# blasif/cocons

Measured on AMD Instinct MI355X. Metric: -2loglik evals/sec (dense cov_rns + Cholesky/solve/log-det, fp64) at n=10000, higher is better.
Workload: dtype f64

## Files before the change

cocons_amd/csrc/api.hip:

```cpp
#include <hip/hip_runtime.h>
#include <limits.h>
#include <math.h>
#include <stdarg.h>
#include <stdint.h>
#include <stdio.h>
#include <stdlib.h>
#include <string.h>
#include <unistd.h>
#include <time.h>
#include <dlfcn.h>
#include <rccl/rccl.h>

#include <algorithm>
#include <limits>
#include <memory>
#include <mutex>
#include <string>
#include <thread>
#include <vector>

#include "kernels.h"
#include "../../include/cocons_hip_diag.h"
#include "matern_device.hpp"

using namespace cocons;

static thread_local std::string g_err;

static int fail(int code, const char *fmt, ...)
{
    char buf[512];
    va_list ap;
    va_start(ap, fmt);
    vsnprintf(buf, sizeof buf, fmt, ap);
    va_end(ap);
    g_err = buf;
    return code;
}

#define HIPCHK(expr)                                                              \
    do {                                                                          \
        hipError_t e__ = (expr);                                                  \
        if (e__ != hipSuccess) {                                                  \
            char b__[512];                                                        \
            snprintf(b__, sizeof b__, "%s failed: %s (%s:%d)", #expr,             \
                     hipGetErrorString(e__), __FILE__, __LINE__);                 \
            g_err = b__;                                                          \
            return -100 - (int)e__;                                               \
        }                                                                         \
    } while (0)

extern "C" const char *cocons_last_error(void) { return g_err.c_str(); }
extern "C" int cocons_abi_version(void) { return 1; }

extern "C" int cocons_device_count(void)
{
    int n = 0;
    hipError_t e = hipGetDeviceCount(&n);
    if (e != hipSuccess) { g_err = hipGetErrorString(e); return -1; }
    return n;
}

extern "C" double cocons_sumsmoothlone(const double *x, int len, double lambda, double alpha)
{
    double sum = 0;
    for (int w = 0; w < len; ++w) {
        if (std::abs(x[w]) > 1e-4)
            sum = sum + std::abs(x[w]);
        else
            sum = sum + std::pow(alpha, -1) * (std::log(1 + std::exp(-alpha * x[w])) + std::log(1 + std::exp(alpha * x[w])));
    }
// ... 1464 lines not shown
    return 0;
}

static int enqueue_eval_impl(cocons_fit *f, const double *theta, const double *mean, bool use_trend,
                             const double *xb, int nxb, std::vector<hipEvent_t> *ev_upd, bool stage_events)
{
    const int nrhs = f->r + nxb;
    f->nrhs_cur = nrhs;
    const int was_clean = f->border_clean;
    const double *was_A = f->dA;
    if (int rc = fit_alloc_matrix(f, nrhs)) return rc;
    const bool zero_rest = !(was_clean == nrhs && was_A == f->dA);
    f->border_pending = nrhs;
    if (stage_events) hipEventRecord(f->ev[0], f->stream);
    if (int rc = reset_info(f)) return rc;
    if (f->taper_nnz > 0) { if (int rc = assemble_sigma_taper(f, theta)) return rc; }
    else assemble_sigma(f, theta, 0, 0, f->npad);
    const bool slots = f->nslot >= nrhs && f->nslot > 0;
    FactorView fv = main_view(f);
    if (slots) fv.mt = fv.nt;
    else fv.trim = (f->rhs_act - nrhs >= 64) ? 1 : 0;
    fv.dag_ok = true;
    if (engine_wanted(f, fv))
        if (int rc = engine_start(f, fv)) return rc;
    assemble_rhs(f, mean, use_trend, xb, nxb, 0, f->npad, zero_rest, slots);
    if (stage_events) hipEventRecord(f->ev[1], f->stream);
    if (int rc = factorize(f, fv, ev_upd)) return rc;
    if (stage_events) hipEventRecord(f->ev[2], f->stream);
    launch_finalize(f->dA, f->lda, f->n, slots ? f->n : f->npad, nrhs, f->dout, f->stream, f->skew, f->npad,
                    f->dag_used ? f->dP : nullptr, f->dag_used ? 2 * TILE * f->dag_nsteps : 0);
    HIPCHK(hipMemcpyAsync(f->hinfo, f->dinfo, (size_t)(2 + nrhs * nrhs) * sizeof(double),
                          hipMemcpyDeviceToHost, f->stream));
    if (stage_events) hipEventRecord(f->ev[3], f->stream);
    HIPCHK(hipGetLastError());
    return 0;
}

static void debug_abort_report(cocons_fit *f)
{
    fprintf(stderr, "cocons: hand-off time-out, code 0x%x\n", f->hinfo[1]);
    const unsigned cls = abort_class((unsigned)f->hinfo[1]);
    if (!f->dag_used || !f->ddag || cls < ABORT_DAG_FIRST || cls > ABORT_DAG_LAST) return;
    unsigned rec[7] = {0, 0, 0, 0, 0, 0, 0}, now = 0, qn = 0;
    hipMemcpyAsync(rec, f->ddag + 8, sizeof rec, hipMemcpyDeviceToHost, f->stream);
    hipStreamSynchronize(f->stream);
    if (rec[2] < f->ddag.count()) hipMemcpyAsync(&now, f->ddag + rec[2], sizeof now, hipMemcpyDeviceToHost, f->stream);
    hipMemcpyAsync(&qn, f->ddag, sizeof qn, hipMemcpyDeviceToHost, f->stream);
    hipStreamSynchronize(f->stream);
    fprintf(stderr, "cocons: DAG wait: task %u (of %u, counter now %u) code 0x%x waited for word %u >= %u, saw %u, holds %u now; "
            "%.1f ms, %u polls\n", rec[0], f->dag_ntasks, qn, rec[1], rec[2], rec[3], rec[4], now, rec[5] * 1e-5, rec[6]);
    if (const char *dump = getenv("COCONS_DEBUG_ABORT_DUMP")) {
        static int ndump = 0;
        char path[512];
        snprintf(path, sizeof path, "%s.%d", dump, ndump++);
        if (FILE *fp = fopen(path, "wb")) {
            const unsigned ntr = f->dag_trace_tasks ? 1u : 0u;
            unsigned hdr[16] = {0xDA6D0001u, (unsigned)f->nt, (unsigned)f->dag_nsteps, f->dag_ntasks, (unsigned)f->ddag.count(),
                                (unsigned)f->flags_cap, ntr, (unsigned)f->hinfo[1], qn, now, 0, 0, 0, 0, 0, 0};
            fwrite(hdr, sizeof hdr, 1, fp);
            fwrite(rec, sizeof rec, 1, fp);
            std::vector<DagStepHost> sh((size_t)f->dag_nsteps);
            hipMemcpyAsync(sh.data(), f->ddag_steps, sh.size() * sizeof(DagStepHost), hipMemcpyDeviceToHost, f->stream);
            std::vector<unsigned> w((size_t)f->ddag.count()), fl(4 * (size_t)f->flags_cap + 64);
            hipMemcpyAsync(w.data(), f->ddag, w.size() * sizeof(unsigned), hipMemcpyDeviceToHost, f->stream);
            hipMemcpyAsync(fl.data(), f->dflags, fl.size() * sizeof(unsigned), hipMemcpyDeviceToHost, f->stream);
            hipStreamSynchronize(f->stream);
// ... 1195 lines not shown
    pa.pad_diag = f->nslot > 0 ? 1e300 : 1.0;
    pa.own_world = world; pa.own_rank = rank; pa.own_group = shard_group();
    launch_pair_sym(ms.mode, false, pa, f->stream);
    const int mt = f->nt + f->rhs_act / TILE;
    if (shard_owner(f->nt / PT, world) == rank)
        assemble_rhs(f, mean, true, nullptr, 0, 0, f->npad);
    launch_front_identity(f->dA, f->lda, f->pad0, mt * TILE, f->stream);
    HIPCHK(hipGetLastError());
    return 0;
}

static int shard_factor_diag(cocons_fit *f, int k)
{
    ShardState *S = f->shard.get();
    const int t = k * PT, w = S->plan.ncols[k] / TILE;
    hipStream_t s = f->stream;
    double *A = f->dA, *q0 = f->dinv, *q1 = f->dinv + 2048;
    if (engine_enabled() && f->flags_cap >= t + w) {
        unsigned *in = f->dflags, *out = f->dflags + f->flags_cap, *xr = f->dflags + 2 * (size_t)f->flags_cap;
        HIPCHK(hipMemsetD32Async((hipDeviceptr_t)(in + t), 7, (size_t)w, s));
        const bool pair = w == 2 && tun().engine_pair && f->dmbox && f->smb_off >= ((size_t)f->nt + 2) * ENGINE_MBOX_DOUBLES;
        launch_potrf_engine(A, f->lda, t, t + w, f->dinv, f->dinfo, in, out, xr, (unsigned *)(f->dinfo + 1),
                            f->dflags + 3 * (size_t)f->flags_cap, s, nullptr, nullptr, 0, nullptr,
                            pair ? f->dmbox : nullptr);
    } else {
        launch_potrf_tile(A, f->lda, t * TILE, q0, f->dinfo, s);
        if (w == 2) {
            launch_trsm_tile(A, f->lda, t * TILE, (t + 1) * TILE, (t + 2) * TILE, q0, s);
            launch_update(A, f->lda, t * TILE, TILE, t + 1, t + 2, t + 1, t + 2, true, s);
            launch_potrf_tile(A, f->lda, (t + 1) * TILE, q1, f->dinfo, s);
        }
    }
    (void)q1;
    double *L = S->lkk[k & 1];
    HIPCHK(hipMemcpy2DAsync(L, (size_t)PT * TILE * sizeof(double), A + (size_t)t * TILE + (size_t)t * TILE * f->lda,
                            f->lda * sizeof(double), (size_t)w * TILE * sizeof(double), (size_t)w * TILE,
                            hipMemcpyDeviceToDevice, s));
    HIPCHK(hipMemcpyAsync(L + (size_t)PT * TILE * PT * TILE, f->dinv, 2 * 2048 * sizeof(double), hipMemcpyDeviceToDevice, s));
    HIPCHK(hipEventRecord(S->ev_main_L, s));
    return 0;
}

static bool shard_comm2()
{
    static const int v = [] { const char *e = getenv("COCONS_SHARD_COMM2"); return e ? atoi(e) : 0; }();
    return v != 0;
}

static int coll_prepare(cocons_fit *f)
{
    if (!f->cstream) HIPCHK(hipStreamCreateWithFlags(&f->cstream, hipStreamNonBlocking));
    if (!f->cstream_l) {
        const bool own = shard_comm2() && (f->coll_kind == 2 || (f->coll_kind == 1 && f->comm_l && f->comm_l != f->comm));
        if (own) HIPCHK(hipStreamCreateWithFlags(&f->cstream_l, hipStreamNonBlocking));
        else f->cstream_l = f->cstream;
    }
    if (!f->dcoll) HIPCHK(f->dcoll.alloc((size_t)(2 + (COCONS_P_MAX + f->r) * (COCONS_P_MAX + f->r))));
    return 0;
}

extern "C" int cocons_comm_unique_id(void *id_out)
{
    if (!id_out) return fail(-1, "cocons_comm_unique_id: null argument");
    RcclApi *R = rccl_api();
    if (!R) return -1;
    ncclUniqueId id;
// ... 92 lines not shown
    const int W = f->coll_world, rank = f->coll_rank, G = shard_group();
    const int t = k * PT, w = P.ncols[k] / TILE, tn = t + w;
    const int mt = P.mt;
    hipStream_t s = f->stream;
    double *A = f->dA;
    if (rank != shard_owner(k, W)) {
        HIPCHK(hipStreamWaitEvent(s, S->ev_comm_L[k & 1], 0));
        const double *L = S->lkk[k & 1];
        HIPCHK(hipMemcpy2DAsync(A + (size_t)t * TILE + (size_t)t * TILE * f->lda, f->lda * sizeof(double), L,
                                (size_t)PT * TILE * sizeof(double), (size_t)w * TILE * sizeof(double), (size_t)w * TILE,
                                hipMemcpyDeviceToDevice, s));
        HIPCHK(hipMemcpyAsync(f->dinv, L + (size_t)PT * TILE * PT * TILE, 2 * 2048 * sizeof(double), hipMemcpyDeviceToDevice, s));
        HIPCHK(hipEventRecord(S->ev_main_U[k & 1], s));
        S->unpacked[k & 1] = true;
    }
    if (tn >= mt) return 0;
    if (P.cnt[(size_t)k * W + rank] > 0) {
        launch_trsm_tile(A, f->lda, t * TILE, tn * TILE, mt * TILE, f->dinv, s, nullptr, nullptr, -1, 0, W, rank, G);
        if (w == 2) {
            launch_update_from(A, f->lda, A + (size_t)t * TILE * f->lda, f->lda, TILE, tn, mt, t + 1, t + 2, false, s, G, W, rank);
            launch_trsm_tile(A, f->lda, (t + 1) * TILE, tn * TILE, mt * TILE, f->dinv + 2048, s, nullptr, nullptr, -1, 0, W, rank, G);
        }
    }
    if (tn >= P.nt) return 0;
    if (k + 1 < nb && rank == shard_owner(k + 1, W)) {
        const int w1 = P.ncols[k + 1] / TILE;
        launch_update(A, f->lda, t * TILE, w * TILE, tn, tn + w1, tn, tn + w1, true, s);
        if (int rc = shard_factor_diag(f, k + 1)) return rc;
    }
    const long long slot = (long long)P.srows[k] * P.ncols[k];
    launch_pack_rows(A, f->lda, t * TILE, w * TILE, f->xbuf[k & 1], (size_t)P.srows[k], S->d_pmap + (size_t)k * 2 * mt, P.tlo[k],
                     2 * mt, slot * rank, slot * (rank + 1), s);
    HIPCHK(hipEventRecord(S->ev_main_X[k & 1], s));
    HIPCHK(hipGetLastError());
    return 0;
}

static int shard_step_post(cocons_fit *f, int k, int nb)
{
    ShardState *S = f->shard.get();
    const ShardPlan &P = S->plan;
    const int W = f->coll_world, rank = f->coll_rank, G = shard_group();
    const int t = k * PT, w = P.ncols[k] / TILE, tn = t + w;
    if (tn >= P.nt) return 0;
    HIPCHK(hipStreamWaitEvent(f->stream, S->ev_comm_X[k & 1], 0));
    if (P.cnt[(size_t)k * W + rank] > 0) {
        const bool ahead = k + 1 < nb && rank == shard_owner(k + 1, W);
        const int skip_lo = ahead ? 2 * tn : 0, skip_hi = ahead ? 2 * (tn + P.ncols[k + 1] / TILE) : 0;
        launch_update_from(f->dA, f->lda, f->xbuf[k & 1], (size_t)P.srows[k], w * TILE, tn, P.mt, tn, P.nt, true, f->stream,
                           G, W, rank, nullptr, -1, nullptr, nullptr, nullptr, -1, 0, 0, 0, 0,
                           S->d_pmap + (size_t)k * 2 * P.mt, skip_lo, skip_hi);
    }
    HIPCHK(hipGetLastError());
    return 0;
}

static int shard_finish(cocons_fit *f, double *partial, int *info)
{
    const int nr = f->nrhs_cur, len = 1 + nr * nr;
    for (int i = 0; i < len; ++i) partial[i] = 0.0;
    const bool mine = shard_owner(f->nt / PT, f->coll_world) == f->coll_rank;
    if (mine) {
        launch_finalize(f->dA, f->lda, f->n, f->npad, nr, f->dout, f->stream);
        HIPCHK(hipMemcpyAsync(f->hout, f->dout, (size_t)len * sizeof(double), hipMemcpyDeviceToHost, f->stream));
    }
    HIPCHK(hipMemcpyAsync(f->hinfo, f->dinfo, 2 * sizeof(int), hipMemcpyDeviceToHost, f->stream));
    HIPCHK(hipStreamSynchronize(f->stream));
    if (mine) for (int i = 0; i < len; ++i) partial[i] = f->hout[i];
    if (info) *info = *f->hinfo;
    return 0;
}

static int sharded_eval_impl(cocons_fit *f, const double *theta, const double *mean, double *sum_logliks, double *parts);

static int sharded_eval(cocons_fit *f, const double *theta, const double *mean, double *sum_logliks, double *parts)
{
    const int rc = sharded_eval_impl(f, theta, mean, sum_logliks, parts);
    if (rc < 0 && f->coll_kind == 1 && f->comm && f->coll_world > 1) {
        const std::string keep = g_err;
        RcclApi *R = rccl_api();
        if (R && f->comm_l && f->comm_l != f->comm) (void)R->CommAbort(f->comm_l);
        if (R) (void)R->CommAbort(f->comm);
        f->comm = nullptr; f->comm_l = nullptr;
        f->coll_kind = -1;
        g_err = keep + " (communicator aborted)";
// ... 343 lines not shown
                                 hipMemcpyDeviceToDevice, M) != hipSuccess) return fail(-100, tiles_failed);
        }
    }
    HIPCHK_AT("cocons_debug_dag_replay", dcmp.alloc(2));
    const size_t T64 = 2 * (size_t)fv.mt;
    unsigned *in = f->dflags, *outw = f->dflags + f->flags_cap, *xr = f->dflags + 2 * (size_t)f->flags_cap;
    unsigned *abort_word = (unsigned *)(f->dinfo + 1);
    unsigned *queue = f->ddag, *tdone = f->ddag + 64, *pdone = tdone + T64 * (T64 + 1) / 2;
    unsigned *pall = pdone + ((size_t)f->dag_nsteps + 2) * T64;
    unsigned *dcount = pall + (size_t)f->dag_nsteps + 64;
    f->upd_flops = 0.0;
    f->nrhs_cur = nrhs;
    for (int s2 = 0; s2 < f->dag_nsteps; ++s2) count_update_flops(f, 2, 2 * s2 + 2);
    const double flops = f->upd_flops;
    HIPCHK_AT("cocons_debug_dag_replay", hipEventCreate(&ev.a));
    HIPCHK_AT("cocons_debug_dag_replay", hipEventCreate(&ev.b));
    double ms_sum = 0.0;
    for (int it = 0; it < reps; ++it) {
        if (int rc = reset_info(f)) return rc;
        assemble_sigma(f, theta, 0, 0, f->npad);
        assemble_rhs(f, mean, true, nullptr, 0, 0, f->npad, true, slots);
        launch_front_identity(fv.A, fv.lda, f->pad0, fv.mt * TILE, M);
        panel_ops(f, fv, 0, M);
        HIPCHK_AT("cocons_debug_dag_replay", hipMemsetAsync(f->ddag, 0, f->ddag.count() * sizeof(unsigned), M));
        HIPCHK_AT("cocons_debug_dag_replay", hipMemsetD32Async((hipDeviceptr_t)f->dflags, 0x3fffffff, 3 * (size_t)f->flags_cap, M));
        unsigned *alive_w = f->dflags + 3 * (size_t)f->flags_cap;
        static const unsigned pair_on_xcd0 = 2u;
        HIPCHK_AT("cocons_debug_dag_replay", hipMemcpyAsync(alive_w + 16, &pair_on_xcd0, sizeof(unsigned), hipMemcpyHostToDevice, M));
        HIPCHK_AT("cocons_debug_dag_replay", hipEventRecord(ev.a, M));
        launch_dag(fv.A, fv.lda, f->dP, f->dWt, f->ddag_steps, f->dag_nsteps, f->dag_ntasks, queue, tdone,
                   pdone, (int)T64, pall, f->dpart, dcount, in, outw, xr, abort_word, M, nullptr, alive_w, dag_xcc_quota(), nullptr,
                   f->dag_have_ftab ? f->ddag_ftab : nullptr, f->dag_xcd_g, f->ddag + f->ddag_xcnt_off);
        HIPCHK_AT("cocons_debug_dag_replay", hipEventRecord(ev.b, M));
        HIPCHK_AT("cocons_debug_dag_replay", hipGetLastError());
        HIPCHK_AT("cocons_debug_dag_replay", hipStreamSynchronize(M));
        float ms = 0;
        HIPCHK_AT("cocons_debug_dag_replay", hipEventElapsedTime(&ms, ev.a, ev.b));
        ms_sum += ms;
    }
    HIPCHK_AT("cocons_debug_dag_replay", hipMemcpyAsync(f->hinfo, f->dinfo, 2 * sizeof(int), hipMemcpyDeviceToHost, M));
    HIPCHK_AT("cocons_debug_dag_replay", hipStreamSynchronize(M));
    if (f->hinfo[1] != 0) return fail(ENGINE_ABORT, "cocons_debug_dag_replay: a wait of the replayed launch ran out");
    HIPCHK_AT("cocons_debug_dag_replay", hipMemsetAsync(dcmp, 0, 2 * sizeof(unsigned long long), M));
    const int c0 = 2 * TILE, c1 = 2 * TILE * f->dag_nsteps, rend = fv.mt * TILE - 64 * fv.trim;
    hipLaunchKernelGGL(panel_diff_kernel, dim3(c1 - c0), dim3(256), 0, M, (const double *)f->dP, (const double *)Lcopy, lda, c0, c1, rend,
                       dcmp.get());
    unsigned long long h[2] = {0, 0};
    HIPCHK_AT("cocons_debug_dag_replay", hipMemcpyAsync(h, dcmp, sizeof h, hipMemcpyDeviceToHost, M));
    HIPCHK_AT("cocons_debug_dag_replay", hipStreamSynchronize(M));
    double md, ml;
    memcpy(&md, &h[0], 8); memcpy(&ml, &h[1], 8);
    out[0] = ms_sum / reps; out[1] = flops; out[2] = ml > 0 ? md / ml : NAN; out[3] = (double)f->dag_ntasks; out[4] = (double)f->dag_nsteps;
    return 0;
}

extern "C" int cocons_debug_dag_replay(cocons_fit *f, const double *theta, const double *mean, int reps, double *out)
{
    FIT_ENTER(f);
    if (int rc = no_taper(f, "cocons_debug_dag_replay")) return rc;
    if (!theta || !mean || !out || reps < 1) return fail(-1, "cocons_debug_dag_replay: bad argument");
    if (f->r < 1 || f->coll_kind) return fail(-1, "cocons_debug_dag_replay: needs a plain dense fit with z");
    const int engine_saved = tun().engine;
    tun().engine = 0;
    int st = enqueue_eval(f, theta, mean, true, nullptr, 0, nullptr, false);
    if (st == 0) { HIPCHK(hipStreamSynchronize(f->stream)); st = info_status(f); }
    tun().engine = engine_saved;
// ... 48 lines not shown
        f->border_clean = -1; f->border_pending = -1;
    }
};

struct TaperGradState {
    DevBuf<double> Z;
    DevBuf<double> AR;
    DevBuf<double> ent;
    DevBuf<double> site;
    DevBuf<double> gsite;
    DevBuf<double> out;
    DevBuf<int> tcp, tidx, trow;
    size_t ldz = 0;
    long long bytes = 0;
};

cocons_fit::cocons_fit() = default;
cocons_fit::~cocons_fit() = default;

static int grad_refuse(cocons_fit *f, const char *who)
{
    if (int rc = no_taper(f, who)) return rc;
    if (f->coll_kind) return fail(-1, "%s: not available on a sharded handle", who);
    return 0;
}

static int grad_contract(cocons_fit *f, const double *theta, int rt, const double *LR, int ncol, double coef, double *hgrad)
{
    const int npad = f->npad, p = f->p;
    hipStream_t s = f->stream;
    GradState *G = f->grad.get();
    launch_grad_fill(f->dA, f->lda, 0, npad, npad, -1, s);
    launch_grad_syrk(f->dA, f->lda, npad, npad + rt, s);
    if (!hgrad) return 0;
    ThetaVecs tv;
    make_theta_vecs(theta, p, tv);
    const ModeSel ms = select_mode(theta, p, f->smooth_limits, 0);
    const int smooth_free = ms.smooth_kind == SMOOTH_LOGISTIC_SQRT && f->smooth_limits[1] != f->smooth_limits[0];
    launch_grad_site(loc_args(f->n, p, f->dX, f->dlocs, G->site, npad, tv, ms.smooth_kind, f->smooth_limits), G->site, npad,
                     smooth_free, s);
    GradArgs g;
    memset(&g, 0, sizeof g);
    g.n = f->n; g.pad0 = f->pad0; g.npad = npad; g.p = p;
    g.S = f->dA; g.lds = f->lda;
    g.AR = LR; g.ldar = npad; g.nr = ncol; g.coef = coef;
    g.loc = f->dloc; g.stride = npad; g.site = G->site;
    g.X = f->dX; g.ldx = f->n;
    g.gr = ms.gr; g.nu_fixed = ms.nu_fixed; g.smooth_free = smooth_free;
    const size_t T = (size_t)npad / 64, ntile = T * (T + 1) / 2;
    g.part_row = G->scratch; g.part_col = g.part_row + ntile * 6 * 64; g.part_glob = g.part_col + ntile * 6 * 64;
    g.gsite = g.part_glob + ntile;
    g.out = G->out;
    launch_grad_pairs(ms.mode, g, s);
    HIPCHK(hipMemcpyAsync(hgrad, G->out, (size_t)7 * p * sizeof(double), hipMemcpyDeviceToHost, s));
    HIPCHK(hipGetLastError());
    return 0;
}

static int grad_enqueue(cocons_fit *f, const double *theta, const double *mean, bool full, double *hgrad)
{
    const int npad = f->npad, nr = f->r, rt = round_up(nr > 0 ? nr : 1, TILE), p = f->p;
    hipStream_t s = f->stream;
    GradState *G = f->grad.get();
    f->nrhs_cur = nr;
    assemble_sigma(f, theta, 0, 0, npad);
    RhsArgs ra;
// ... 373 lines not shown
```

cocons_amd/csrc/chol.hip:

```cpp
#include <hip/hip_runtime.h>
#include <limits.h>
#include <stdlib.h>
#include <string.h>
#include <algorithm>
#include <atomic>
#include <vector>
#include "kernels.h"

namespace cocons {

typedef double d4 __attribute__((ext_vector_type(4)));

#define MFMA64(a, b, c) __builtin_amdgcn_mfma_f64_16x16x4f64((a), (b), (c), 0, 0, 0)
#define MFMA64_NEGA(a, b, c) __builtin_amdgcn_mfma_f64_16x16x4f64((a), (b), (c), 0, 0, 1)
#define LDS_T __attribute__((address_space(3)))

__device__ __forceinline__ void blk_mma(d4 &acc, const d4 &P, const d4 &Q)
{
    acc = MFMA64(Q[0], P[0], acc);
    acc = MFMA64(Q[1], P[1], acc);
    acc = MFMA64(Q[2], P[2], acc);
    acc = MFMA64(Q[3], P[3], acc);
}

// ... 1228 lines not shown
        double Q[4];
#pragma unroll
        for (int s = 0; s < 4; ++s) Q[s] = QS[j * 256 + s * 64 + lane];
        trsm16(B[j], L, Q);
        d4 NX = -B[j];
#pragma unroll
        for (int jj = j + 1; jj < 8; ++jj) {
            d4 Lb = lds_blk(SL + (jj * (jj + 1) / 2 + j) * 256, lane);
            blk_mma(B[jj], NX, Lb);
        }
    }
#pragma unroll
    for (int j = 0; j < 8; ++j) glb_blk_store(A, lda, rs, c0 + 16 * j, lane, B[j]);
}


struct UpdArgs {
    double *C; size_t ldc;
    const double *P; size_t ldp;
    int K;
    int ti0, tj0, lower_only;
    int H, W;
    unsigned *sig; int sig_tile;
    unsigned *wait_word, *abort_word;
    int ptiles, world, rank;
    const int *pmap;
    int skip_lo, skip_hi;
    unsigned *queue; unsigned ntiles;
    int Hb, ext0;
    int c_wt;
    int skew, kblk;
};

template <int TM, int KC, int ROLE, int NW = 4>
__global__ void __launch_bounds__(64 * NW, 8)
update_kernel(UpdArgs a)
{
    constexpr int LDT = TM + 16;
    constexpr int WY = NW / 2;
    constexpr int NB = TM / 32;
    constexpr int NBY = TM / WY / 16;
    constexpr int TPC = 64 * NW / KC;
    constexpr int RPT = TM / TPC;
    __shared__ double sI[2][KC * LDT];
    __shared__ double sJ[2][KC * LDT];
    unsigned *share = (unsigned *)&sI[0][TM];
    const int tid = threadIdx.x;
    const int wave_s = __builtin_amdgcn_readfirstlane(tid >> 6);
    if (a.wait_word) {
        if (tid == 0) *share = wait_ge(a.wait_word, 1u, a.abort_word, abort_code(ABORT_INPANEL, (unsigned)a.tj0)) ? 1u : 0u;
        asm volatile("s_waitcnt vmcnt(0)" ::: "memory");
        __syncthreads();
        const unsigned ok = *share;
        __syncthreads();
        if (!ok) return;
    }

    else if (a.abort_word) {
        if (tid == 0) *share = __hip_atomic_load(a.abort_word, __ATOMIC_RELAXED, __HIP_MEMORY_SCOPE_AGENT);
        __syncthreads();
        const unsigned ab = *share;
        __syncthreads();
        if (ab) return;
    }

    const int nch = a.K / KC;
    typedef double d2 __attribute__((ext_vector_type(2)));

    unsigned L = blockIdx.x;
    for (;;) {
        int lane;
        asm volatile("v_mbcnt_lo_u32_b32 %0, -1, 0\n\tv_mbcnt_hi_u32_b32 %0, -1, %0" : "=v"(lane));
        const int wave = wave_s, t2 = 64 * wave + lane;
        const int wi = wave & 1, wj = wave >> 1;
        const int kc = t2 / TPC, rg = (t2 % TPC) * RPT;
        const int ro = (lane >> 4) * LDT + (lane & 15);
        int ti, tj;
        if (a.lower_only) {
            int lo = 0, hi = a.W - 1;
            while (lo < hi) {
                const int mid = (lo + hi + 1) >> 1;
                if (mid * a.H - mid * (mid - 1) / 2 <= (int)L) lo = mid; else hi = mid - 1;
            }
            const int j = lo;
            const int til = j + ((int)L - (j * a.H - j * (j - 1) / 2));
            tj = a.tj0 + j;
            ti = til < a.Hb ? a.tj0 + til : a.ext0 + (til - a.Hb);
        } else {
            const int til = blockIdx.x;
            ti = til < a.Hb ? a.ti0 + til : a.ext0 + (til - a.Hb);
            tj = a.tj0 + blockIdx.y;
        }
        if (a.world > 1 && ((ti * TM / (2 * TILE) / a.ptiles) % a.world) != a.rank) return;
        if (ti >= a.skip_lo && ti < a.skip_hi && tj >= a.skip_lo && tj < a.skip_hi) {
            if (!a.queue) return;
            if (t2 == 0) *share = gridDim.x + __hip_atomic_fetch_add(a.queue, 1u, __ATOMIC_RELAXED, __HIP_MEMORY_SCOPE_AGENT);
            __syncthreads();
            L = (unsigned)__builtin_amdgcn_readfirstlane((int)*share);
            __syncthreads();
            if (L >= a.ntiles) break;
            continue;
        }
        const int sig_Ti = (ti * TM) / TILE - a.sig_tile, sig_Tj = (tj * TM) / TILE - a.sig_tile;
        const bool sig_wg = a.sig != nullptr && sig_Ti >= 0 && sig_Ti <= 1 && sig_Tj >= 0 && sig_Tj <= sig_Ti;
        const bool wt_wg = sig_wg || a.c_wt;
        if (sig_wg) __builtin_amdgcn_s_setprio(3); else __builtin_amdgcn_s_setprio(0);

        int rowI_P = ti * TM, rowJ_P = tj * TM, rowI_C = ti * TM;
        if (a.pmap) { rowI_P = a.pmap[ti]; rowJ_P = a.pmap[tj]; }
        if (a.skew) {
            const bool ext = ti >= a.ext0;
            const int under = a.skew * TILE + (ti - a.ext0) * TM;
            rowI_P = ext ? under : ti * TM - TILE * a.kblk;
            rowJ_P = tj * TM - TILE * a.kblk;
            rowI_C = ext ? under : ti * TM - TILE * ((tj * TM) / TILE);
        }
        const double *gI = a.P + (size_t)(rowI_P + rg) + (size_t)kc * a.ldp;
        const double *gJ = a.P + (size_t)(rowJ_P + rg) + (size_t)kc * a.ldp;
        d2 stI[RPT / 2], stJ[RPT / 2];

        double *Cb = a.C + (size_t)(rowI_C + (TM / 2) * wi) + (size_t)(tj * TM + (TM / WY) * wj) * a.ldc;
        const unsigned ldcb = 8u * (unsigned)a.ldc;
        const unsigned cvo = 8u * (unsigned)(lane & 15) + (unsigned)(lane >> 4) * ldcb;
        d4 acc[NB][NBY];
#pragma unroll
        for (int x = 0; x < NB; ++x)
#pragma unroll
            for (int y = 0; y < NBY; ++y) acc[x][y] = (d4){0.0, 0.0, 0.0, 0.0};

#pragma unroll
        for (int v = 0; v < RPT / 2; ++v) {
            stI[v] = *(const d2 *)(gI + 2 * v);
            stJ[v] = *(const d2 *)(gJ + 2 * v);
        }
#pragma unroll
        for (int v = 0; v < RPT / 2; ++v) {
            *(d2 *)(&sI[0][kc * LDT + rg + 2 * v]) = stI[v];
            *(d2 *)(&sJ[0][kc * LDT + rg + 2 * v]) = stJ[v];
        }
        __syncthreads();

        for (int ch = 0; ch < nch; ++ch) {
            const int cur = ch & 1;
            if (ch + 1 < nch) {
                const double *pI = gI + (size_t)(ch + 1) * KC * a.ldp;
                const double *pJ = gJ + (size_t)(ch + 1) * KC * a.ldp;
#pragma unroll
                for (int v = 0; v < RPT / 2; ++v) {
                    stI[v] = *(const d2 *)(pI + 2 * v);
                    stJ[v] = *(const d2 *)(pJ + 2 * v);
                }
            }
            const double *bI = &sI[cur][ro + (TM / 2) * wi];
            const double *bJ = &sJ[cur][ro + (TM / WY) * wj];
#pragma unroll
            for (int s = 0; s < KC / 4; ++s) {
                double pi_[NB], pj_[NBY];
#pragma unroll
                for (int x = 0; x < NB; ++x) pi_[x] = bI[s * 4 * LDT + 16 * x];
#pragma unroll
                for (int y = 0; y < NBY; ++y) pj_[y] = bJ[s * 4 * LDT + 16 * y];
#pragma unroll
                for (int x = 0; x < NB; ++x)
#pragma unroll
                    for (int y = 0; y < NBY; ++y) acc[x][y] = MFMA64(pj_[y], pi_[x], acc[x][y]);
            }
            if (ch + 1 < nch) {
#pragma unroll
                for (int v = 0; v < RPT / 2; ++v) {
                    *(d2 *)(&sI[cur ^ 1][kc * LDT + rg + 2 * v]) = stI[v];
                    *(d2 *)(&sJ[cur ^ 1][kc * LDT + rg + 2 * v]) = stJ[v];
                }
            }
            __syncthreads();
        }
        unsigned Lnext = 0;
        if (a.queue && t2 == 0)
            Lnext = gridDim.x + __hip_atomic_fetch_add(a.queue, 1u, __ATOMIC_RELAXED, __HIP_MEMORY_SCOPE_AGENT);
        unsigned cve = cvo;
        asm volatile("" : "+v"(cve));
#pragma unroll
        for (int x = 0; x < NB; ++x)
#pragma unroll
            for (int y = 0; y < NBY; ++y) {
                d4 cv;
#pragma unroll
                for (int r = 0; r < 4; ++r) {
                    const double *cp = (const double *)((const char *)(Cb + 16 * x) + (cve + (unsigned)(16 * y + 4 * r) * ldcb));
                    cv[r] = a.c_wt ? load_wt(cp) : *cp;
                }
                cv -= acc[x][y];
                if (wt_wg) {
#pragma unroll
                    for (int r = 0; r < 4; ++r)
                        store_wt((double *)((char *)(Cb + 16 * x) + (cve + (unsigned)(16 * y + 4 * r) * ldcb)), cv[r]);
                } else {
#pragma unroll
                    for (int r = 0; r < 4; ++r)
                        *(double *)((char *)(Cb + 16 * x) + (cve + (unsigned)(16 * y + 4 * r) * ldcb)) = cv[r];
                }
            }
        if (wt_wg) {
            asm volatile("s_waitcnt vmcnt(0)" ::: "memory");
            __syncthreads();
            if (t2 == 0 && sig_wg) signal_add(a.sig + a.sig_tile + sig_Ti);
        }
        if (!a.queue) break;
        if (t2 == 0) *share = Lnext;
        __syncthreads();
        L = (unsigned)__builtin_amdgcn_readfirstlane((int)*share);
        if (L >= a.ntiles) break;
    }
}

struct DagStep {
    unsigned base;
    unsigned near;
    unsigned tpos, nT;
    int H, W;
    int tj0;
    int k0, K;
    int nstrip, two;
    int need;
    int nd_next;
    int split;
    unsigned p2, p3;
};

struct DagArgs {
    double *A; size_t lda;
    double *P;
    const double *Wt;
    const DagStep *steps; int nsteps;
    unsigned ntasks;
    unsigned *queue;
    unsigned *tdone;
    unsigned *pdone; int pstride;
    unsigned *pall;
    double *partbuf;
    unsigned *dcount;
    unsigned *sig;
    unsigned *out, *xr;
    unsigned *abort_word;
    const unsigned *alive;
    unsigned xcc_quota;
// ... 687 lines not shown
}

void launch_potrf_follow(double *A, size_t lda, int c0, int r0, int r1, double *dinv, int *info, double *mbox,
                         unsigned *abort_word, hipStream_t s, int band_r1, int ext_r0)
{
    int nb1 = ((band_r1 >= 0 ? band_r1 : r1) - r0) / 64, nb2 = band_r1 >= 0 ? (r1 - ext_r0) / 64 : 0;
    if (nb1 < 0) nb1 = 0;
    if (nb2 < 0) nb2 = 0;
    const int nstrips = nb1 + nb2;
    static std::atomic<unsigned long long> attr_done{0};
    const size_t shm = 76 * 1024;
    set_dynamic_lds_once((const void *)potrf_follow_kernel, shm, attr_done);
    hipLaunchKernelGGL(potrf_follow_kernel, dim3(1 + (nstrips + 1) / 2), dim3(512), shm, s, A, lda, c0, dinv, info, mbox, r0, nb1,
                       ext_r0, nstrips, abort_word);
}

void launch_panel_pair(double *A, size_t lda, int c0, int r0, int r1, unsigned *xr, unsigned *abort_word, hipStream_t s,
                       const double *mb0, const double *mb1, double *smb, int ndiag, unsigned *sig, int sig_tile, double *xmb)
{
    const int nb = (r1 - r0) / 64;
    if (nb <= 0) return;
    const bool split = xmb != nullptr;
    const bool diag = smb && ndiag > 0 && nb >= (ndiag == 10 ? 4 : 2);
    hipLaunchKernelGGL(panel_pair_kernel, dim3((split ? 2 * nb : nb) + (diag ? ndiag : 0)), dim3(256), 0, s, A, lda, c0, r0,
                       xr, abort_word, mb0, mb1, diag ? smb : nullptr, nb, diag ? (ndiag == 10 ? 4 : 2) : 0, sig, sig_tile, xmb);
}

static int upd_waves = -1;
static long long upd_w8_max_tiles = -1;
void set_update_waves(int nw) { upd_waves = nw == 8 ? 8 : 4; }
void set_update_w8_max_tiles(int ntiles) { upd_w8_max_tiles = ntiles < 0 ? 0 : ntiles; }
static int upd_c_wt = 0;
void set_update_c_wt(int on) { upd_c_wt = on ? 1 : 0; }

void launch_update_from(double *A, size_t lda, const double *P, size_t ldp, int K,
                        int ti0, int ti1, int tj0, int tj1, bool lower_only, hipStream_t s,
                        int ptiles, int world, int rank, unsigned *sig, int sig_tile,
                        unsigned *wait_word, unsigned *abort_word, unsigned *queue, int band_hi, int ext0,
                        int skew, int kblk, int trim64, const int *pmap, int skip_lo, int skip_hi)
{
    const bool band = band_hi >= 0;
    const int rows_band = (band ? band_hi : ti1) - ti0, rows_ext = band ? ti1 - ext0 : 0;
    if (rows_band + rows_ext <= 0 || rows_band < 0 || rows_ext < 0 || tj1 <= tj0 || K <= 0) return;
    trim64 = trim64 ? 1 : 0;
    const int rows64 = 2 * (rows_band + rows_ext) - trim64;
    if (rows64 <= 0) return;
    if (upd_waves < 0) { const char *e = getenv("COCONS_UPD_WAVES"); set_update_waves(e ? atoi(e) : 8); }
    if (upd_w8_max_tiles < 0) { const char *e = getenv("COCONS_UPD_W8_MAX_TILES"); set_update_w8_max_tiles(e ? atoi(e) : 3500); }
    bool use_w8 = false;
    UpdArgs a;
    a.queue = nullptr; a.ntiles = 0;
    a.skew = skew; a.kblk = kblk; a.c_wt = upd_c_wt;
    a.Hb = 2 * rows_band; a.ext0 = 2 * ext0;
    a.C = A; a.ldc = lda; a.P = P; a.ldp = ldp; a.K = K;
    a.lower_only = lower_only ? 1 : 0;
    a.ptiles = ptiles < 1 ? 1 : ptiles; a.world = world; a.rank = rank; a.pmap = pmap; a.skip_lo = skip_lo; a.skip_hi = skip_hi;
    a.sig = sig; a.sig_tile = sig_tile;
    a.wait_word = wait_word; a.abort_word = abort_word;
    a.H = 0; a.W = 0;
    a.ti0 = 2 * ti0; a.tj0 = 2 * tj0;
    dim3 grid(rows64, 2 * (tj1 - tj0));
    if (lower_only) {
        if (ti0 != tj0) { a.lower_only = 0; }
        else {
            const long long H = rows64, W = 2LL * (tj1 - tj0);
            a.H = (int)H; a.W = (int)W;
            const long long total = W * H - W * (W - 1) / 2;
            static int slots = 0;
            if (!slots) {
                int dev = 0, cus = 256;
                hipGetDevice(&dev);
                hipDeviceGetAttribute(&cus, hipDeviceAttributeMultiprocessorCount, dev);
                slots = 8 * cus;
            }
            grid = dim3((unsigned)total, 1);
            if (queue && world == 1) {
                const bool w8 = upd_waves == 8 && K >= 2 * TILE && !skew &&
                                (upd_w8_max_tiles == 0 || total <= upd_w8_max_tiles);
                use_w8 = w8;
                const int cap = w8 ? slots / 2 - 4 : slots - 8;
                if (total > cap + (w8 ? 4 : 8)) {
                    a.queue = queue; a.ntiles = (unsigned)total;
                    grid = dim3((unsigned)cap, 1);
                }
            }
        }
    }
    const bool trailing = (K > TILE) && world == 1;
    if (trailing && use_w8 && a.lower_only) hipLaunchKernelGGL((update_kernel<64, 16, 0, 8>), grid, dim3(512), 0, s, a);
    else if (trailing) hipLaunchKernelGGL((update_kernel<64, 8, 0>), grid, dim3(256), 0, s, a);
    else hipLaunchKernelGGL((update_kernel<64, 8, 1>), grid, dim3(256), 0, s, a);
}

__global__ void __launch_bounds__(256)
pack_rows_kernel(const double *A, size_t lda, int col0, int ncols, double *dst, size_t ldp, const int *pmap, int ti_lo,
                 long long slot_lo, long long slot_hi)
{
    const int ti = ti_lo + (int)blockIdx.x;
    const long long off = pmap[ti];
    if (off < slot_lo || off >= slot_hi) return;
    const int rho = threadIdx.x & 63, cq = threadIdx.x >> 6;
    for (int c = 4 * (int)blockIdx.y + cq; c < ncols; c += 4 * (int)gridDim.y)
        dst[off + rho + (size_t)c * ldp] = A[(size_t)(64 * ti + rho) + (size_t)(col0 + c) * lda];
}

void launch_pack_rows(const double *A, size_t lda, int col0, int ncols, double *dst, size_t ldp, const int *pmap, int ti_lo,
                      int ti_hi, long long slot_lo, long long slot_hi, hipStream_t s)
{
    if (ti_hi <= ti_lo || ncols <= 0) return;
    hipLaunchKernelGGL(pack_rows_kernel, dim3(ti_hi - ti_lo, 8), dim3(256), 0, s, A, lda, col0, ncols, dst, ldp, pmap, ti_lo,
// ... 374 lines not shown
```

cocons_amd/csrc/kernels.h:

```cpp
#pragma once
#include <hip/hip_runtime.h>
#include <stddef.h>
#include <vector>
#include "../../include/cocons_hip.h"

namespace cocons {

enum SmoothKind : int {
    SMOOTH_ZERO = 0,
    SMOOTH_LOGISTIC_SQRT = 1,
    SMOOTH_EXP = 2
};

struct ThetaVecs {
    double tilt[COCONS_P_MAX];
    double two_scale_je[COCONS_P_MAX];
    double aniso[COCONS_P_MAX];
    double sqrt_vector[COCONS_P_MAX];
    double half_sd[COCONS_P_MAX];
    double nugget[COCONS_P_MAX];
    double smooth[COCONS_P_MAX];
    double sd[COCONS_P_MAX];
};

// ... 71 lines not shown
                         double *wbuf = nullptr, double *pbuf = nullptr, int dag_until = 0,
                         unsigned long long *trace = nullptr,
                         double *mbox = nullptr,
                         int in_wait_ms = 0);
constexpr unsigned ABORT_ENGINE_IN0 = 0x100u, ABORT_ENGINE_IN1 = 0x200u, ABORT_PANEL = 0x300u, ABORT_XCHG = 0x400u, ABORT_INPANEL = 0x500u,
                   ABORT_GATE = 0x600u, ABORT_PARTNER = 0x700u, ABORT_FOLLOW = 0x800u, ABORT_LAST_TILE = 0x900u, ABORT_STRIPBOX = 0xf00u,
                   ABORT_DAG_FIRST = 0xa00u, ABORT_DAG_LAST = 0xe00u;
__host__ __device__ inline unsigned abort_code(unsigned cls, unsigned index) { return cls | (index & 0xffu); }
inline unsigned abort_class(unsigned code) { return code & 0xf00u; }
constexpr size_t ENGINE_MBOX_DOUBLES = 44 * 256;
void launch_engine_gate(unsigned *alive, unsigned *abort_word, hipStream_t s, bool last_tile = false, bool patient = false, int nhelp = 0,
                        unsigned *raise_in = nullptr);
void launch_raise_word(unsigned *word, hipStream_t s);
int streams_run_concurrently(hipStream_t first, hipStream_t second, unsigned *words);
void launch_trsm_tile(double *A, size_t lda, int c0, int r0, int r1, const double *dinv, hipStream_t s,
                      unsigned *wait_word = nullptr, unsigned *abort_word = nullptr, int band_r1 = -1, int ext_r0 = 0,
                      int own_world = 0, int own_rank = 0, int own_group = 1);
void launch_panel_pair(double *A, size_t lda, int c0, int r0, int r1, unsigned *xr, unsigned *abort_word, hipStream_t s,
                       const double *mb0, const double *mb1,
                       double *smb = nullptr, int ndiag = 0, unsigned *sig = nullptr, int sig_tile = 0,
                       double *xmb = nullptr);
constexpr size_t PANEL_XMBOX_DOUBLES = 8 * 4 * 256;
constexpr size_t PANEL_SMBOX_DOUBLES = 4 * 16 * 4 * 256;
void launch_update(double *A, size_t lda, int k0, int K, int ti0, int ti1, int tj0, int tj1,
                   bool lower_only, hipStream_t s, unsigned *sig = nullptr, int sig_tile = -1,
                   unsigned *wait_word = nullptr, unsigned *abort_word = nullptr, unsigned *queue = nullptr,
                   int band_hi = -1, int ext0 = 0,
                   int skew = 0,
                   int trim64 = 0,
                   int skip_lo = 0, int skip_hi = 0);
void set_update_waves(int nw);
void set_update_w8_max_tiles(int ntiles);
void set_update_c_wt(int on);
void launch_update_from(double *A, size_t lda, const double *P, size_t ldp, int K,
                        int ti0, int ti1, int tj0, int tj1, bool lower_only, hipStream_t s,
                        int group, int world, int rank, unsigned *sig = nullptr, int sig_tile = -1,
                        unsigned *wait_word = nullptr, unsigned *abort_word = nullptr, unsigned *queue = nullptr,
                        int band_hi = -1, int ext0 = 0, int skew = 0, int kblk = 0, int trim64 = 0,
                        const int *pmap = nullptr, int skip_lo = 0, int skip_hi = 0);
void launch_pack_rows(const double *A, size_t lda, int col0, int ncols, double *dst, size_t ldp, const int *pmap, int ti_lo,
                      int ti_hi, long long slot_lo, long long slot_hi, hipStream_t s);

struct DagStepHost {
    unsigned base, near, tpos, nT;
    int H, W, tj0, k0, K, nstrip, two, need, nd_next, split;
    unsigned p2, p3;
};
unsigned dag_build_steps(int nt, int mt, int trim64, int kskip, int lead, int min_tiles, std::vector<DagStepHost> &out,
                         int lead2 = 0, int lead3 = 0,
                         std::vector<unsigned> *ftab = nullptr,
                         int xcd_g = 0, int bw = 16, int bh = 16);
void launch_dag(double *A, size_t lda, double *P, const double *Wt, const DagStepHost *dsteps, int nsteps, unsigned ntasks,
                unsigned *queue, unsigned *tdone, unsigned *pdone, int pstride, unsigned *pall, double *partbuf, unsigned *dcount,
                unsigned *sig, unsigned *out, unsigned *xr, unsigned *abort_word, hipStream_t s, unsigned long long *trace = nullptr,
                const unsigned *alive = nullptr, int xcc_quota = 0, unsigned *hw = nullptr,
                const unsigned *ftab = nullptr, int xcd_g = 0,
                unsigned *xcnt = nullptr);

void launch_finalize(const double *A, size_t lda, int n, int row0, int nr, double *out, hipStream_t s,
                     int skew = 0, int npad = 0,
                     const double *A2 = nullptr,
                     int a2_cols = 0);
void launch_finalize_cols(const double *A, size_t lda, int c0, int c1, int n, int row0, int nr,
                          double *out, hipStream_t s);
size_t row_reduce_scratch_doubles(int n, int m);
void launch_row_reduce(const double *A, size_t lda, int n, int rowy, int row0, int m,
// ... 71 lines not shown
```

Baseline: 124.1.

## Stream update-kernel panels into LDS via async DMA ring and prefetch next tile

Rewrites the trailing-update GEMM kernel to load panel chunks directly into a 4-stage LDS ring with global_load_lds, replacing the register-staged double buffer. The kernel also fetches the next persistent-queue tile and primes its first stages during the C write-back of the current tile, so loads overlap compute and epilogue. It adds alignment and K-multiple requirements, reported through a new refusal check, and depends on hand-placed waitcnt and barrier sequencing, which risks races.

```diff
diff --git a/cocons_amd/csrc/api.hip b/cocons_amd/csrc/api.hip
--- a/cocons_amd/csrc/api.hip
+++ b/cocons_amd/csrc/api.hip
@@ -37,6 +37,11 @@
     g_err = buf;
     return code;
 }
+
+#define UPDCHK()                                                                  \
+    do {                                                                          \
+        if (const char *m__ = take_update_refusal()) return fail(-1, "%s", m__);  \
+    } while (0)
 
 #define HIPCHK(expr)                                                              \
     do {                                                                          \
@@ -1567,6 +1572,7 @@
     HIPCHK(hipMemcpyAsync(f->hinfo, f->dinfo, (size_t)(2 + nrhs * nrhs) * sizeof(double),
                           hipMemcpyDeviceToHost, f->stream));
     if (stage_events) hipEventRecord(f->ev[3], f->stream);
+    UPDCHK();
     HIPCHK(hipGetLastError());
     return 0;
 }
@@ -2828,6 +2834,7 @@
         }
     }
     (void)q1;
+    UPDCHK();
     double *L = S->lkk[k & 1];
     HIPCHK(hipMemcpy2DAsync(L, (size_t)PT * TILE * sizeof(double), A + (size_t)t * TILE + (size_t)t * TILE * f->lda,
                             f->lda * sizeof(double), (size_t)w * TILE * sizeof(double), (size_t)w * TILE,
@@ -2986,6 +2993,7 @@
     launch_pack_rows(A, f->lda, t * TILE, w * TILE, f->xbuf[k & 1], (size_t)P.srows[k], S->d_pmap + (size_t)k * 2 * mt, P.tlo[k],
                      2 * mt, slot * rank, slot * (rank + 1), s);
     HIPCHK(hipEventRecord(S->ev_main_X[k & 1], s));
+    UPDCHK();
     HIPCHK(hipGetLastError());
     return 0;
 }
@@ -3005,6 +3013,7 @@
                            G, W, rank, nullptr, -1, nullptr, nullptr, nullptr, -1, 0, 0, 0, 0,
                            S->d_pmap + (size_t)k * 2 * P.mt, skip_lo, skip_hi);
     }
+    UPDCHK();
     HIPCHK(hipGetLastError());
     return 0;
 }
@@ -3414,6 +3423,7 @@
                    pdone, (int)T64, pall, f->dpart, dcount, in, outw, xr, abort_word, M, nullptr, alive_w, dag_xcc_quota(), nullptr,
                    f->dag_have_ftab ? f->ddag_ftab : nullptr, f->dag_xcd_g, f->ddag + f->ddag_xcnt_off);
         HIPCHK_AT("cocons_debug_dag_replay", hipEventRecord(ev.b, M));
+        UPDCHK();
         HIPCHK_AT("cocons_debug_dag_replay", hipGetLastError());
         HIPCHK_AT("cocons_debug_dag_replay", hipStreamSynchronize(M));
         float ms = 0;
@@ -3528,6 +3538,7 @@
     GradState *G = f->grad.get();
     launch_grad_fill(f->dA, f->lda, 0, npad, npad, -1, s);
     launch_grad_syrk(f->dA, f->lda, npad, npad + rt, s);
+    UPDCHK();
     if (!hgrad) return 0;
     ThetaVecs tv;
     make_theta_vecs(theta, p, tv);
diff --git a/cocons_amd/csrc/chol.hip b/cocons_amd/csrc/chol.hip
--- a/cocons_amd/csrc/chol.hip
+++ b/cocons_amd/csrc/chol.hip
@@ -1284,19 +1284,69 @@
     int skew, kblk;
 };
 
+struct UpdTile {
+    int ti, tj;
+    int rowI_P, rowJ_P, rowI_C;
+};
+
+template <int TM>
+__device__ __forceinline__ UpdTile upd_tile(const UpdArgs &a, unsigned L)
+{
+    UpdTile t;
+    if (a.lower_only) {
+        int lo = 0, hi = a.W - 1;
+        while (lo < hi) {
+            const int mid = (lo + hi + 1) >> 1;
+            if (mid * a.H - mid * (mid - 1) / 2 <= (int)L) lo = mid; else hi = mid - 1;
+        }
+        const int j = lo;
+        const int til = j + ((int)L - (j * a.H - j * (j - 1) / 2));
+        t.tj = a.tj0 + j;
+        t.ti = til < a.Hb ? a.tj0 + til : a.ext0 + (til - a.Hb);
+    } else {
+        const int til = blockIdx.x;
+        t.ti = til < a.Hb ? a.ti0 + til : a.ext0 + (til - a.Hb);
+        t.tj = a.tj0 + blockIdx.y;
+    }
+    t.rowI_P = t.ti * TM; t.rowJ_P = t.tj * TM; t.rowI_C = t.ti * TM;
+    if (a.pmap) {
+        t.rowI_P = __builtin_amdgcn_readfirstlane(a.pmap[t.ti]);
+        t.rowJ_P = __builtin_amdgcn_readfirstlane(a.pmap[t.tj]);
+    }
+    if (a.skew) {
+        const bool ext = t.ti >= a.ext0;
+        const int under = a.skew * TILE + (t.ti - a.ext0) * TM;
+        t.rowI_P = ext ? under : t.ti * TM - TILE * a.kblk;
+        t.rowJ_P = t.tj * TM - TILE * a.kblk;
+        t.rowI_C = ext ? under : t.ti * TM - TILE * ((t.tj * TM) / TILE);
+    }
+    return t;
+}
+
+__device__ __forceinline__ int fresh_lane()
+{
+    int lane;
+    asm volatile("v_mbcnt_lo_u32_b32 %0, -1, 0\n\tv_mbcnt_hi_u32_b32 %0, -1, %0" : "=v"(lane));
+    return lane;
+}
+
+__device__ __forceinline__ bool upd_skipped(const UpdArgs &a, const UpdTile &t)
+{
+    return t.ti >= a.skip_lo && t.ti < a.skip_hi && t.tj >= a.skip_lo && t.tj < a.skip_hi;
+}
+
 template <int TM, int KC, int ROLE, int NW = 4>
 __global__ void __launch_bounds__(64 * NW, 8)
 update_kernel(UpdArgs a)
 {
-    constexpr int LDT = TM + 16;
+    constexpr int KS = KC / 2;
+    constexpr int RING = 4, STG = 2 * KS * TM;
     constexpr int WY = NW / 2;
     constexpr int NB = TM / 32;
     constexpr int NBY = TM / WY / 16;
-    constexpr int TPC = 64 * NW / KC;
-    constexpr int RPT = TM / TPC;
-    __shared__ double sI[2][KC * LDT];
-    __shared__ double sJ[2][KC * LDT];
-    unsigned *share = (unsigned *)&sI[0][TM];
+    static_assert(TM == 64 && KS == NW && KS % 4 == 0, "one DMA per wave and stage: two 64-row columns of one operand");
+    __shared__ double smem[RING * STG + 2];
+    unsigned *share = (unsigned *)&smem[RING * STG];
     const int tid = threadIdx.x;
     const int wave_s = __builtin_amdgcn_readfirstlane(tid >> 6);
     if (a.wait_word) {
@@ -1316,121 +1366,104 @@
         if (ab) return;
     }
 
-    const int nch = a.K / KC;
-    typedef double d2 __attribute__((ext_vector_type(2)));
+    const int nch = a.K / KS;
+
+    const int wave = wave_s;
+    const int wi = wave & 1, wj = wave >> 1;
+    const bool opJ = wave >= NW / 2;
+    const unsigned ldpb = 8u * (unsigned)a.ldp, cstep = (unsigned)KS * ldpb;
+    auto src_offset = [&]() -> unsigned {
+        const int l = fresh_lane(), sc = (l >> 5) & 1;
+        return (unsigned)(2 * (wave % (NW / 2)) + sc) * ldpb + 8u * (unsigned)((2 * (l & 31)) ^ (16 * sc));
+    };
+    LDS_T double *ldst = (LDS_T double *)(smem + 128 * wave);
+#define UPD_STAGE(slot)                                                                                                     \
+    do {                                                                                                                    \
+        __builtin_amdgcn_global_load_lds((const void *)src, (LDS_T void *)(ldst + STG * (slot)), 16, 0, 0);                 \
+        src += cstep;                                                                                                       \
+    } while (0)
+    const unsigned ldcb = 8u * (unsigned)a.ldc;
 
     unsigned L = blockIdx.x;
+    UpdTile T = upd_tile<TM>(a, L);
+    bool primed = false;
+    const char *src = nullptr;
     for (;;) {
-        int lane;
-        asm volatile("v_mbcnt_lo_u32_b32 %0, -1, 0\n\tv_mbcnt_hi_u32_b32 %0, -1, %0" : "=v"(lane));
-        const int wave = wave_s, t2 = 64 * wave + lane;
-        const int wi = wave & 1, wj = wave >> 1;
-        const int kc = t2 / TPC, rg = (t2 % TPC) * RPT;
-        const int ro = (lane >> 4) * LDT + (lane & 15);
-        int ti, tj;
-        if (a.lower_only) {
-            int lo = 0, hi = a.W - 1;
-            while (lo < hi) {
-                const int mid = (lo + hi + 1) >> 1;
-                if (mid * a.H - mid * (mid - 1) / 2 <= (int)L) lo = mid; else hi = mid - 1;
-            }
-            const int j = lo;
-            const int til = j + ((int)L - (j * a.H - j * (j - 1) / 2));
-            tj = a.tj0 + j;
-            ti = til < a.Hb ? a.tj0 + til : a.ext0 + (til - a.Hb);
-        } else {
-            const int til = blockIdx.x;
-            ti = til < a.Hb ? a.ti0 + til : a.ext0 + (til - a.Hb);
-            tj = a.tj0 + blockIdx.y;
-        }
-        if (a.world > 1 && ((ti * TM / (2 * TILE) / a.ptiles) % a.world) != a.rank) return;
-        if (ti >= a.skip_lo && ti < a.skip_hi && tj >= a.skip_lo && tj < a.skip_hi) {
-            if (!a.queue) return;
-            if (t2 == 0) *share = gridDim.x + __hip_atomic_fetch_add(a.queue, 1u, __ATOMIC_RELAXED, __HIP_MEMORY_SCOPE_AGENT);
-            __syncthreads();
-            L = (unsigned)__builtin_amdgcn_readfirstlane((int)*share);
-            __syncthreads();
-            if (L >= a.ntiles) break;
-            continue;
-        }
-        const int sig_Ti = (ti * TM) / TILE - a.sig_tile, sig_Tj = (tj * TM) / TILE - a.sig_tile;
+        if (!primed) {
+            if (a.world > 1 && ((T.ti * TM / (2 * TILE) / a.ptiles) % a.world) != a.rank) return;
+            if (upd_skipped(a, T)) {
+                if (!a.queue) return;
+                if (threadIdx.x == 0) *share = gridDim.x + __hip_atomic_fetch_add(a.queue, 1u, __ATOMIC_RELAXED, __HIP_MEMORY_SCOPE_AGENT);
+                __syncthreads();
+                L = (unsigned)__builtin_amdgcn_readfirstlane((int)*share);
+                __syncthreads();
+                if (L >= a.ntiles) break;
+                T = upd_tile<TM>(a, L);
+                continue;
+            }
+            src = (const char *)(a.P + (opJ ? T.rowJ_P : T.rowI_P)) + src_offset();
+            UPD_STAGE(0);
+            UPD_STAGE(1);
+            UPD_STAGE(2);
+        }
+        const int sig_Ti = (T.ti * TM) / TILE - a.sig_tile, sig_Tj = (T.tj * TM) / TILE - a.sig_tile;
         const bool sig_wg = a.sig != nullptr && sig_Ti >= 0 && sig_Ti <= 1 && sig_Tj >= 0 && sig_Tj <= sig_Ti;
         const bool wt_wg = sig_wg || a.c_wt;
         if (sig_wg) __builtin_amdgcn_s_setprio(3); else __builtin_amdgcn_s_setprio(0);
 
-        int rowI_P = ti * TM, rowJ_P = tj * TM, rowI_C = ti * TM;
-        if (a.pmap) { rowI_P = a.pmap[ti]; rowJ_P = a.pmap[tj]; }
-        if (a.skew) {
-            const bool ext = ti >= a.ext0;
-            const int under = a.skew * TILE + (ti - a.ext0) * TM;
-            rowI_P = ext ? under : ti * TM - TILE * a.kblk;
-            rowJ_P = tj * TM - TILE * a.kblk;
-            rowI_C = ext ? under : ti * TM - TILE * ((tj * TM) / TILE);
-        }
-        const double *gI = a.P + (size_t)(rowI_P + rg) + (size_t)kc * a.ldp;
-        const double *gJ = a.P + (size_t)(rowJ_P + rg) + (size_t)kc * a.ldp;
-        d2 stI[RPT / 2], stJ[RPT / 2];
-
-        double *Cb = a.C + (size_t)(rowI_C + (TM / 2) * wi) + (size_t)(tj * TM + (TM / WY) * wj) * a.ldc;
-        const unsigned ldcb = 8u * (unsigned)a.ldc;
-        const unsigned cvo = 8u * (unsigned)(lane & 15) + (unsigned)(lane >> 4) * ldcb;
+        int aI[NB], aJ[NBY];
+        {
+            const int lane = fresh_lane(), kq = lane >> 4, kodd = kq & 1;
+#pragma unroll
+            for (int x = 0; x < NB; ++x) aI[x] = TM * kq + (((TM / 2) * wi + 16 * x + (lane & 15)) ^ (16 * kodd));
+#pragma unroll
+            for (int y = 0; y < NBY; ++y) aJ[y] = KS * TM + TM * kq + (((TM / WY) * wj + 16 * y + (lane & 15)) ^ (16 * kodd));
+        }
+        double *Cb = a.C + (size_t)(T.rowI_C + (TM / 2) * wi) + (size_t)(T.tj * TM + (TM / WY) * wj) * a.ldc;
         d4 acc[NB][NBY];
 #pragma unroll
         for (int x = 0; x < NB; ++x)
 #pragma unroll
             for (int y = 0; y < NBY; ++y) acc[x][y] = (d4){0.0, 0.0, 0.0, 0.0};
 
-#pragma unroll
-        for (int v = 0; v < RPT / 2; ++v) {
-            stI[v] = *(const d2 *)(gI + 2 * v);
-            stJ[v] = *(const d2 *)(gJ + 2 * v);
-        }
-#pragma unroll
-        for (int v = 0; v < RPT / 2; ++v) {
-            *(d2 *)(&sI[0][kc * LDT + rg + 2 * v]) = stI[v];
-            *(d2 *)(&sJ[0][kc * LDT + rg + 2 * v]) = stJ[v];
-        }
-        __syncthreads();
-
-        for (int ch = 0; ch < nch; ++ch) {
-            const int cur = ch & 1;
-            if (ch + 1 < nch) {
-                const double *pI = gI + (size_t)(ch + 1) * KC * a.ldp;
-                const double *pJ = gJ + (size_t)(ch + 1) * KC * a.ldp;
-#pragma unroll
-                for (int v = 0; v < RPT / 2; ++v) {
-                    stI[v] = *(const d2 *)(pI + 2 * v);
-                    stJ[v] = *(const d2 *)(pJ + 2 * v);
-                }
-            }
-            const double *bI = &sI[cur][ro + (TM / 2) * wi];
-            const double *bJ = &sJ[cur][ro + (TM / WY) * wj];
-#pragma unroll
-            for (int s = 0; s < KC / 4; ++s) {
-                double pi_[NB], pj_[NBY];
-#pragma unroll
-                for (int x = 0; x < NB; ++x) pi_[x] = bI[s * 4 * LDT + 16 * x];
-#pragma unroll
-                for (int y = 0; y < NBY; ++y) pj_[y] = bJ[s * 4 * LDT + 16 * y];
-#pragma unroll
-                for (int x = 0; x < NB; ++x)
-#pragma unroll
-                    for (int y = 0; y < NBY; ++y) acc[x][y] = MFMA64(pj_[y], pi_[x], acc[x][y]);
-            }
-            if (ch + 1 < nch) {
-#pragma unroll
-                for (int v = 0; v < RPT / 2; ++v) {
-                    *(d2 *)(&sI[cur ^ 1][kc * LDT + rg + 2 * v]) = stI[v];
-                    *(d2 *)(&sJ[cur ^ 1][kc * LDT + rg + 2 * v]) = stJ[v];
-                }
-            }
-            __syncthreads();
-        }
+#define UPD_STEP(r, WAIT, ISSUE)                                                                                            \
+        do {                                                                                                                \
+            WAIT;                                                                                                           \
+            asm volatile("s_waitcnt lgkmcnt(0)" ::: "memory");                                                              \
+            __builtin_amdgcn_s_barrier();                                                                                   \
+            asm volatile("" ::: "memory");                                                                                  \
+            if (ISSUE) UPD_STAGE(((r) + RING - 1) % RING);                                                                  \
+            const double *bs = smem + STG * (r);                                                                            \
+            _Pragma("unroll") for (int s = 0; s < KS / 4; ++s) {                                                            \
+                double pi_[NB], pj_[NBY];                                                                                   \
+                _Pragma("unroll") for (int x = 0; x < NB; ++x) pi_[x] = bs[s * 4 * TM + aI[x]];                             \
+                _Pragma("unroll") for (int y = 0; y < NBY; ++y) pj_[y] = bs[s * 4 * TM + aJ[y]];                            \
+                _Pragma("unroll") for (int x = 0; x < NB; ++x)                                                              \
+                    _Pragma("unroll") for (int y = 0; y < NBY; ++y) acc[x][y] = MFMA64(pj_[y], pi_[x], acc[x][y]);          \
+            }                                                                                                               \
+        } while (0)
+#define UPD_VM(n) asm volatile("s_waitcnt vmcnt(" #n ")" ::: "memory")
+        UPD_STEP(0, if (!primed) UPD_VM(2), true);
+        UPD_STEP(1, if (!primed) UPD_VM(2), true);
+        UPD_STEP(2, if (!primed) UPD_VM(2), true);
+        UPD_STEP(3, UPD_VM(2), true);
+        for (int c0 = RING; c0 < nch - RING; c0 += RING) {
+            UPD_STEP(0, UPD_VM(2), true);
+            UPD_STEP(1, UPD_VM(2), true);
+            UPD_STEP(2, UPD_VM(2), true);
+            UPD_STEP(3, UPD_VM(2), true);
+        }
+        UPD_STEP(0, UPD_VM(2), true);
+        UPD_STEP(1, UPD_VM(2), false);
+        UPD_STEP(2, UPD_VM(1), false);
+        UPD_STEP(3, UPD_VM(0), false);
+#undef UPD_VM
+#undef UPD_STEP
+        const int le = fresh_lane(), t2 = 64 * wave + le;
         unsigned Lnext = 0;
-        if (a.queue && t2 == 0)
-            Lnext = gridDim.x + __hip_atomic_fetch_add(a.queue, 1u, __ATOMIC_RELAXED, __HIP_MEMORY_SCOPE_AGENT);
-        unsigned cve = cvo;
-        asm volatile("" : "+v"(cve));
+        UpdTile Tn = T;
+        bool pf = false;
+        const unsigned cve = 8u * (unsigned)(le & 15) + (unsigned)(le >> 4) * ldcb;
 #pragma unroll
         for (int x = 0; x < NB; ++x)
 #pragma unroll
@@ -1441,6 +1474,25 @@
                     const double *cp = (const double *)((const char *)(Cb + 16 * x) + (cve + (unsigned)(16 * y + 4 * r) * ldcb));
                     cv[r] = a.c_wt ? load_wt(cp) : *cp;
                 }
+                if (x == 0 && y == 0 && a.queue) {
+                    if (t2 == 0)
+                        *share = gridDim.x + __hip_atomic_fetch_add(a.queue, 1u, __ATOMIC_RELAXED, __HIP_MEMORY_SCOPE_AGENT);
+                    asm volatile("s_waitcnt lgkmcnt(0)" ::: "memory");
+                    __builtin_amdgcn_s_barrier();
+                    asm volatile("" ::: "memory");
+                    Lnext = (unsigned)__builtin_amdgcn_readfirstlane((int)*share);
+                    if (Lnext < a.ntiles) {
+                        Tn = upd_tile<TM>(a, Lnext);
+                        if (!upd_skipped(a, Tn)) {
+                            pf = true;
+                            src = (const char *)(a.P + (opJ ? Tn.rowJ_P : Tn.rowI_P)) + src_offset();
+                            UPD_STAGE(0);
+                            UPD_STAGE(1);
+                            UPD_STAGE(2);
+                        }
+                    }
+                }
+                if (x == NB - 1 && y == NBY - 1) asm volatile("s_waitcnt vmcnt(0)" ::: "memory");
                 cv -= acc[x][y];
                 if (wt_wg) {
 #pragma unroll
@@ -1458,11 +1510,12 @@
             if (t2 == 0 && sig_wg) signal_add(a.sig + a.sig_tile + sig_Ti);
         }
         if (!a.queue) break;
-        if (t2 == 0) *share = Lnext;
-        __syncthreads();
-        L = (unsigned)__builtin_amdgcn_readfirstlane((int)*share);
+        L = Lnext;
         if (L >= a.ntiles) break;
-    }
+        T = Tn;
+        primed = pf;
+    }
+#undef UPD_STAGE
 }
 
 struct DagStep {
@@ -2216,6 +2269,8 @@
 void set_update_w8_max_tiles(int ntiles) { upd_w8_max_tiles = ntiles < 0 ? 0 : ntiles; }
 static int upd_c_wt = 0;
 void set_update_c_wt(int on) { upd_c_wt = on ? 1 : 0; }
+static std::atomic<const char *> upd_refusal{nullptr};
+const char *take_update_refusal() { return upd_refusal.exchange(nullptr); }
 
 void launch_update_from(double *A, size_t lda, const double *P, size_t ldp, int K,
                         int ti0, int ti1, int tj0, int tj1, bool lower_only, hipStream_t s,
@@ -2229,6 +2284,10 @@
     trim64 = trim64 ? 1 : 0;
     const int rows64 = 2 * (rows_band + rows_ext) - trim64;
     if (rows64 <= 0) return;
+    if (((uintptr_t)P & 15u) != 0 || (ldp & 1u) != 0 || K % 16 != 0 || K < 32) {
+        upd_refusal.store("launch_update_from: the panel must be 16-byte aligned with an even column stride, K a multiple of 16 >= 32");
+        return;
+    }
     if (upd_waves < 0) { const char *e = getenv("COCONS_UPD_WAVES"); set_update_waves(e ? atoi(e) : 8); }
     if (upd_w8_max_tiles < 0) { const char *e = getenv("COCONS_UPD_W8_MAX_TILES"); set_update_w8_max_tiles(e ? atoi(e) : 3500); }
     bool use_w8 = false;
@@ -2259,7 +2318,7 @@
             }
             grid = dim3((unsigned)total, 1);
             if (queue && world == 1) {
-                const bool w8 = upd_waves == 8 && K >= 2 * TILE && !skew &&
+                const bool w8 = upd_waves == 8 && K >= 2 * TILE && K % 32 == 0 && !skew &&
                                 (upd_w8_max_tiles == 0 || total <= upd_w8_max_tiles);
                 use_w8 = w8;
                 const int cap = w8 ? slots / 2 - 4 : slots - 8;
diff --git a/cocons_amd/csrc/kernels.h b/cocons_amd/csrc/kernels.h
--- a/cocons_amd/csrc/kernels.h
+++ b/cocons_amd/csrc/kernels.h
@@ -127,6 +127,7 @@
 void set_update_waves(int nw);
 void set_update_w8_max_tiles(int ntiles);
 void set_update_c_wt(int on);
+const char *take_update_refusal();
 void launch_update_from(double *A, size_t lda, const double *P, size_t ldp, int K,
                         int ti0, int ti1, int tj0, int tj1, bool lower_only, hipStream_t s,
                         int group, int world, int rank, unsigned *sig = nullptr, int sig_tile = -1,
```

After: 124.7 (median of 4 runs). No clear change (+0.6%).
